# robin-karlsson0/pc-accumulation-lib

Measured on AMD Instinct MI355X. Metric: Mpoints/s projected+accumulated and BEV frames/s @256x256; 1/2/4/8 GPU, higher is better.
Workload: dtype f64; 1 GPU; KITTI-360 single forward cam, 120k pts/frame, 200 m horizon (~201 live frames, 5169634 stored pts), one 256x256x21 BEV per integrated frame; points_per_frame=120000, bev_px=256, view_m=80

## Files before the change

### pc-accumulation-lib_amd/csrc/pca_api.hip

```cpp
#include <stdio.h>
#include <cmath>
#include "pca_common.h"

__global__ __launch_bounds__(256) void pca_fetch_block_kernel(const uint4 *src, uint4 *dst, int64_t n16)
{
    for (int64_t i = (int64_t)blockIdx.x * 256 + threadIdx.x; i < n16; i += (int64_t)gridDim.x * 256) dst[i] = src[i];
}

int pca_fetch_block(pca_ctx *ctx, const void *mapped_host, int64_t offset, void *dev, int64_t bytes, hipStream_t s)
{
    if (bytes <= 0) return 0;
    void *src = nullptr;
    PCA_CHECK(ctx, hipHostGetDevicePointer(&src, const_cast<void *>(mapped_host), 0));
    src = reinterpret_cast<char *>(src) + offset;
    const int64_t n16 = (bytes + 15) / 16;
    const int grid = (int)((n16 + 255) / 256 < 64 ? (n16 + 255) / 256 : 64);
    hipLaunchKernelGGL(pca_fetch_block_kernel, dim3(grid), dim3(256), 0, s, reinterpret_cast<const uint4 *>(src),
                       reinterpret_cast<uint4 *>(dev), n16);
    PCA_CHECK(ctx, hipGetLastError());
    return 0;
}

int pca_ctx_reserve_tiles(pca_ctx *ctx, int64_t tiles, hipStream_t s)
{
// ... 107 lines not shown
                    const double ua = s * (row[0] * cone[0] + row[1] * cone[1] + row[2] * cone[2] + q[axis]);
                    bool out = ua >= h;
                    for (int k = 0; k < 4 && out; ++k) {
                        const double *d = cone + 3 + 3 * k;
                        out = s * (row[0] * d[0] + row[1] * d[1] + row[2] * d[2]) >= 0.0;
                    }
                    if (out) return false;
                }
                if (box) {
                    const float *b = box + 6 * (size_t)f;
                    if (b[0] <= b[1] && b[2] <= b[3] && b[4] <= b[5]) {
                        double lo = s * q[axis];
                        for (int c = 0; c < 3; ++c) {
                            const double x0 = s * row[c] * (double)b[2 * c], x1 = s * row[c] * (double)b[2 * c + 1];
                            lo += x0 < x1 ? x0 : x1;
                        }
                        if (lo >= h) return false;
                    }
                }
            }
        return true;
    };
    int a = 0, b = F - 1;
    while (a <= b && !visible(a)) ++a;
    while (b >= a && !visible(b)) --b;
    if (a > b) { *first = -1; *last = -1; } else { *first = a; *last = b; }
    return 0;
}

int pca_bev_view_hint(pca_ctx *ctx, int slot0, int F, const double *then, const float *box, const double *cone, const double now[12],
                      const pca_bev_params *prm)
{
    if (!ctx) return -1;
    int first = 0, last = 0;
    if (pca_host_view_hull(F, then, box, cone, now, prm, &first, &last)) return -1;
    if (first == 0 && last == F - 1) return 0;
    if (first < 0) { first = 0; last = -1; }
    ctx->bin_first = slot0 + first; ctx->bin_end = slot0 + last + 1; ctx->bin_valid = true;
    return 1;
}

int pca_bev_bin_range(pca_ctx *ctx, int slot_first, int slot_last_plus1)
{
    if (!ctx) return -1;
    ctx->bin_first = slot_first; ctx->bin_end = slot_last_plus1; ctx->bin_valid = slot_last_plus1 >= slot_first;
    return 0;
}

static inline bool box_inside(double x, double y, double lo, double hi) { return lo < x && x < hi && lo < y && y < hi; }

int pca_host_ego_to_grid(const double *full, int F, const double R[9], double dx, double dy, double view, int px,
                         double *rows, int32_t *start)
{
    if (F < 2) { if (F == 1 && start) start[0] = 0; return 0; }
    const double h = 0.5 * view, lo = -h, pxd = (double)px, half_px = 0.5 * pxd;
    auto rot = [&](const double *p, double &x, double &y, double &z) {
        x = fma(R[2], p[2], fma(R[1], p[1], R[0] * p[0])) + dx;
        y = fma(R[5], p[2], fma(R[4], p[1], R[3] * p[0])) + dy;
        z = fma(R[8], p[2], fma(R[7], p[1], R[6] * p[0]));
    };
    auto emit = [&](int m, double x, double y, double z) {
        rows[3 * m + 0] = floor(x / view * pxd + half_px);
        rows[3 * m + 1] = floor(y / view * pxd + half_px);
        rows[3 * m + 2] = z;
    };
    int m = 0;
// ... 151 lines not shown
```

### pc-accumulation-lib_amd/csrc/pca_bev.hip

```cpp
#include "pca_bev_common.h"
#include "pca_k1_body.h"
#include <cstdlib>
#include <mutex>

#define KEY_INVALID 0xffffffffu
#define TS 8
#define TCELLS (TS * TS)
#define NFK (2 * TCELLS)
#ifndef AB_THREADS
#define AB_THREADS 1024
#endif
#define MAX_G 512
#ifndef BIN_RUNR
#define BIN_RUNR 4
#endif
#ifndef BIN_WPE
#define BIN_WPE 4
#endif
#ifndef BIN_UNR
#define BIN_UNR 4
#endif
#ifndef BIN_REG_P
#define BIN_REG_P 12
#endif
// ... 2 lines not shown
#endif
#define C_WAVES (C_THREADS / 64)
#define C_HIST_WAVES 4
#define RGB_CAP 4096
#define CONTIG_MIN 2560
#define HEAVY_MIN_DEFAULT 2560
#define FLAG_ROAD (1u << 24)
#define FLAG_DYNOBJ (1u << 25)

struct __attribute__((aligned(16))) RecF { double z; uint32_t iw; uint32_t cw; };
struct RecD { double z; double inten; uint32_t c; uint32_t fk; };

struct alignas(16) BevArgs {
    pca_store st;
    const double *intensity64;
    const int64_t *frame_off;
    int slot_begin, slot_split, slot_end;
    int64_t max_points;
    pca_bev_params prm;
    int n_pend;
    int write_back;
    int pend_slot_end[PCA_BEV_MAX_CHAIN];
    Mat34 pend_T[PCA_BEV_MAX_CHAIN];
    int tx, T, G;
    int Gr, Gp;
    int tile_mult;
    int heavy_min;
    int stagger;
    uint32_t *key;
    uint32_t *bh;
    uint32_t *boff;
    int Gk;
    int bin_first, bin_end;
    int k1_slot, k1_n;
    uint32_t *bh0;
    int split;
    uint32_t *heavy_hint;
    uint32_t heavy_hint_known;
    uint32_t *span_hint;
    uint32_t span_hint_known;
    int heavy_launched;
    uint32_t *heavy;
    void *recs;
    double *planes;
    uint16_t *planes_f16;
    double *extra;
    uint32_t *status;
    int dbg;
    int band_r0, band_rows;
};
#define HQ_CLASSES 32
#define HQ_CURSOR 32
#define HQ_DONE 33
#define HQ_IDS 64

struct Window { int64_t lo, hi, sp, c_lo, c_hi; };

__device__ __forceinline__ int chunk_index(const BevArgs &a, int64_t lo, int64_t sp, int64_t chunk)
{
    (void)a; (void)lo; (void)sp; (void)chunk;
    return (int)blockIdx.x;
}
#define K1_SEG 4096
#define K1_RIDE 32
__device__ __forceinline__ int64_t window_end(const BevArgs &a)
{
// ... 167 lines not shown
    const int gp = table_pos(a, g);
    uint32_t sum = 0;
    if (split) { for (int k = 0; k < per; ++k) sum += t0 + k < a.T ? s_h[2 * (t0 + k)] + s_h[2 * (t0 + k) + 1] : 0u; }
    else { for (int k = 0; k < per; ++k) sum += t0 + k < a.T ? s_h[t0 + k] : 0u; }
    const int lane = threadIdx.x & 63, wave = threadIdx.x >> 6;
    const uint32_t inc = wave_incl_scan_add(sum);
    if (lane == 63) s_wsum[wave] = inc;
    __syncthreads();
    uint32_t before = 0;
    for (int k = 0; k < wave; ++k) before += s_wsum[k];
    uint32_t run = before + inc - sum;
    for (int k = 0; k < per; ++k) {
        const int t = t0 + k;
        if (t >= a.T) break;
        if (split) {
            const uint32_t c0 = s_h[2 * t], c1 = s_h[2 * t + 1];
            s_cur[2 * t] = run;
            s_cur[2 * t + 1] = run + c0;
            a.bh[(int64_t)t * a.Gr + gp] = c0 + c1;
            a.boff[(int64_t)t * a.Gr + gp] = run;
            a.bh0[(int64_t)t * a.Gr + gp] = c0;
            run += c0 + c1;
        } else {
            const uint32_t c = s_h[t];
            s_cur[t] = run;
            a.bh[(int64_t)t * a.Gr + gp] = c;
            a.boff[(int64_t)t * a.Gr + gp] = run;
            run += c;
        }
    }
}
}

template <bool I64, bool BAND = false>
__device__ __forceinline__ void bev_tile_bin_body(const BevArgs &a)
{
    constexpr int REG_P = I64 ? 0 : BIN_REG_P;
    constexpr int UNR = BIN_RUNR;
    extern __shared__ uint32_t s_lds[];
    __shared__ uint32_t s_wsum[AB_THREADS / 64];
    __shared__ uint32_t s_dyn[8];
    uint32_t *s_h = s_lds;
    if (threadIdx.x < 8) {
        uint32_t w = (uint32_t)a.prm.dynobj_mask[0];
#pragma unroll
        for (int i = 1; i < 8; ++i) w = (int)threadIdx.x == i ? (uint32_t)(a.prm.dynobj_mask[i >> 1] >> (32 * (i & 1))) : w;
        s_dyn[threadIdx.x] = w;
    }
    BIN_STAMP(0);
    int g;
    const Window w = chunk_of(a, g);
    const int64_t chunk = seg_stride(w.hi - w.lo, a.G - a.Gk);
    const bool split = bev_split(a, w.hi - w.lo);
    const int hs = split ? 6 : 7;
    const int n_hist = split ? 2 * a.T : a.T;
    uint32_t *s_cur = s_lds + n_hist;
    if ((int)blockIdx.x == a.Gk) {
        const int64_t end_ub = a.Gk ? a.frame_off[a.k1_slot] + a.k1_n : a.frame_off[a.slot_end];
        if (threadIdx.x == 0 && end_ub - a.frame_off[a.slot_begin] > a.max_points + a.k1_n) pca_raise(a.status, PCA_STATUS_STORE_OVERFLOW);
        if (threadIdx.x < HQ_IDS) a.heavy[threadIdx.x] = 0;
        if (threadIdx.x == 0 && a.span_hint) {
            const uint32_t kp = (uint32_t)((w.hi - w.lo + 1023) >> 10);
            if (kp != a.span_hint_known) *a.span_hint = kp;
        }
    }
    for (int t = threadIdx.x; t < n_hist; t += AB_THREADS) s_h[t] = 0;
// ... 140 lines not shown
    BIN_STAMP(4);
    const bool stale = a.n_pend > 0 && !a.write_back;
    for (int64_t base = reg_hi + threadIdx.x; base < w.c_hi; base += MUNR * AB_THREADS) {
        uint32_t key[MUNR], pos[MUNR], rgbs[MUNR];
        double zz[MUNR], iv[MUNR], xs[MUNR], ys[MUNR];
#pragma unroll
        for (int u = 0; u < MUNR; ++u) {
            const int64_t p = base + u * AB_THREADS;
            key[u] = p < w.c_hi ? a.key[p - w.lo] : KEY_INVALID;
        }
#pragma unroll
        for (int u = 0; u < MUNR; ++u) {
            const int64_t p = base + u * AB_THREADS;
            const bool ok = key[u] != KEY_INVALID;
            rgbs[u] = ok ? a.st.rgbs[p] : 0u;
            zz[u] = ok ? a.st.z[p] : 0.0;
            xs[u] = (ok && stale) ? a.st.x[p] : 0.0;
            ys[u] = (ok && stale) ? a.st.y[p] : 0.0;
            if (I64) iv[u] = ok ? a.intensity64[p] : 0.0;
            else iv[u] = ok ? (double)a.st.intensity[p] : 0.0;
        }
#pragma unroll
        for (int u = 0; u < MUNR; ++u) {
            const int64_t p = base + u * AB_THREADS;
            const bool ok = key[u] != KEY_INVALID;
            if (ok && stale) apply_owed(a, pend_hi, p, xs[u], ys[u], zz[u]);
            pos[u] = ok ? seg + atomicAdd(&s_cur[key[u] >> hs], 1u) : 0u;
        }
#pragma unroll
        for (int u = 0; u < MUNR; ++u)
            if (key[u] != KEY_INVALID) bin_store<I64>(a, s_dyn, pos[u], key[u], rgbs[u], zz[u], iv[u], (float)iv[u]);
    }
    BIN_STAMP(5);
    if ((a.dbg & 32) && threadIdx.x == 0 && blockIdx.x < 1024) { g_dbg_stamps[blockIdx.x][6] = (unsigned long long)a.n_pend * 2 + a.write_back; g_dbg_stamps[blockIdx.x][7] = __smid(); }
}

struct RecMap {
    uint32_t pre[1024 + 1];
    uint32_t base[1024];
    uint32_t wsum[16];
};
__device__ __forceinline__ uint32_t recmap_build(RecMap &M, const BevArgs &a, int tile, int nthreads, uint16_t *owner = nullptr, int half = -1)
{
    const int per = (a.Gr + nthreads - 1) / nthreads;
    const int g0 = threadIdx.x * per;
    const uint32_t *cnt = a.bh + (int64_t)tile * a.Gr, *off = a.boff + (int64_t)tile * a.Gr;
    uint32_t c[4] = {0, 0, 0, 0}, o[4] = {0, 0, 0, 0}, c0[4] = {0, 0, 0, 0}, sum = 0;
    int grp[4] = {0, 0, 0, 0};
#pragma unroll
    for (int k = 0; k < 4; ++k)
        if (k < per && g0 + k < a.Gr) {
            grp[k] = table_group(a, g0 + k);
            if (grp[k] < a.G) {
                c[k] = cnt[g0 + k]; o[k] = off[g0 + k];
                if (half >= 0) c0[k] = a.bh0[(int64_t)tile * a.Gr + g0 + k];
            }
        }
    const int64_t lo = window_begin(a), hi0 = window_end(a);
    const int64_t n = hi0 - lo > a.max_points ? a.max_points : hi0 - lo;
    if (half >= 0 && bev_split(a, n)) {
#pragma unroll
        for (int k = 0; k < 4; ++k) { if (half == 0) c[k] = c0[k]; else { o[k] += c0[k]; c[k] -= c0[k]; } }
    }
    const uint32_t chunk = (uint32_t)seg_stride(n, a.G - a.Gk);
#pragma unroll
    for (int k = 0; k < 4; ++k)
// ... 948 lines not shown
#define BAND_TILES 16384
static inline int band_rows(int px) { const int tx = tiles_x(px); return tx * tx <= BAND_TILES ? tx : BAND_TILES / tx; }
static int bev_tile_mult(int Tp)
{
    auto gcd = [](int x, int y) { while (y) { const int t = x % y; x = y; y = t; } return x; };
    int m = (int)(Tp * 0.6180339887) | 1;
    while (m > 1 && gcd(m, Tp) != 1) m -= 2;
    return m < 1 ? 1 : m;
}
static void bev_set_band(BevArgs &a, int r0)
{
    const int rows = band_rows(a.prm.px);
    a.band_r0 = r0;
    a.band_rows = a.tx - r0 < rows ? a.tx - r0 : rows;
    a.T = a.band_rows * a.tx;
    a.tile_mult = bev_tile_mult(a.T);
}
static inline int max_groups()
{
    const char *e = getenv("PCA_BEV_G");
    const int max_g = e ? atoi(e) : MAX_G;
    return (max_g < 1 || max_g > 1024) ? MAX_G : max_g;
}
static inline int n_groups(int64_t max_points)
{
    const char *c = getenv("PCA_BEV_CHUNK");
    const int max_g = max_groups();
    int per_g = c ? atoi(c) : 8192;
    if (per_g < 1024) per_g = 8192;
    int64_t g = (max_points + per_g - 1) / per_g;
    return (int)(g < 1 ? 1 : (g > max_g ? max_g : g));
}

extern "C" {

int64_t pca_bev_workspace_bytes(int64_t max_points, int px)
{
    if (max_points < 1) max_points = 1;
    const int64_t T = (int64_t)band_rows(px) * tiles_x(px), G = n_groups(max_points);
    return align256(max_points * 4) + 3 * align256((G + K1_RIDE + 8) * T * 4) + align256((HQ_IDS + HQ_CLASSES * T) * 4) +
           align256((max_points + G + K1_RIDE + K1_SEG) * 24) + 512;
}

int pca_bev_generate(pca_ctx *ctx, const pca_store *store, const double *intensity64, const int64_t *frame_off,
                     int slot_begin, int slot_split, int slot_end, int64_t max_points, const pca_bev_params *prm,
                     const double *pending_T, int pending_slot_end, void *workspace, int64_t workspace_bytes,
                     double *planes, uint16_t *planes_f16, void *stream)
{
    return pca_bev_generate_ex(ctx, store, intensity64, frame_off, slot_begin, slot_split, slot_end, max_points, prm,
                               pending_T, pending_slot_end, workspace, workspace_bytes, planes, planes_f16, nullptr, stream);
}

int pca_bev_generate_ex(pca_ctx *ctx, const pca_store *store, const double *intensity64, const int64_t *frame_off,
                        int slot_begin, int slot_split, int slot_end, int64_t max_points, const pca_bev_params *prm,
                        const double *pending_T, int pending_slot_end, void *workspace, int64_t workspace_bytes,
                        double *planes, uint16_t *planes_f16, double *extra_planes, void *stream)
{
    const int n = (pending_T && pending_slot_end > slot_begin) ? 1 : 0;
    return pca_bev_generate_chain(ctx, store, intensity64, frame_off, slot_begin, slot_split, slot_end, max_points, prm,
                                  pending_T, &pending_slot_end, n, 1, workspace, workspace_bytes, planes, planes_f16,
                                  extra_planes, stream);
}

static void bev_table_order(BevArgs &a)
{
    static int xt = -1;
// ... 20 lines not shown
    if (!(slot_begin <= slot_split && slot_split <= slot_end)) { ctx->err = "bev: need slot_begin <= slot_split <= slot_end"; return -1; }
    if (max_points >= (1ll << 32)) { ctx->err = "bev: window too large for 32-bit positions"; return -1; }
    if (workspace_bytes < pca_bev_workspace_bytes(max_points, prm->px)) { ctx->err = "bev: workspace too small"; return -1; }
    a.st = *store;
    a.intensity64 = intensity64;
    a.frame_off = frame_off;
    a.slot_begin = slot_begin; a.slot_split = slot_split; a.slot_end = slot_end;
    a.max_points = max_points;
    a.prm = *prm;
    a.n_pend = n_pending;
    a.write_back = write_back ? 1 : 0;
    for (int k = 0; k < PCA_BEV_MAX_CHAIN; ++k) {
        a.pend_slot_end[k] = slot_begin;
        for (int i = 0; i < 12; ++i) a.pend_T[k].m[i] = 0.0;
        if (k >= n_pending) continue;
        if (pending_slot_ends[k] > slot_end) { ctx->err = "bev: a pending slot end lies beyond the window"; return -1; }
        if (k > 0 && pending_slot_ends[k] < pending_slot_ends[k - 1]) { ctx->err = "bev: pending slot ends must ascend"; return -1; }
        a.pend_slot_end[k] = pending_slot_ends[k];
        for (int i = 0; i < 12; ++i) a.pend_T[k].m[i] = pending_Ts[16 * k + i];
    }
    a.tx = tiles_x(prm->px);
    a.band_rows = band_rows(prm->px);
    a.band_r0 = 0;
    a.T = a.band_rows * a.tx;
    a.G = n_groups(max_points);
    bev_table_order(a);
    char *w = reinterpret_cast<char *>((reinterpret_cast<uintptr_t>(workspace) + 255) & ~(uintptr_t)255);
    a.key = reinterpret_cast<uint32_t *>(w); w += align256(max_points * 4);
    a.bh = reinterpret_cast<uint32_t *>(w); w += align256((int64_t)(a.G + K1_RIDE + 8) * a.T * 4);
    a.boff = reinterpret_cast<uint32_t *>(w); w += align256((int64_t)(a.G + K1_RIDE + 8) * a.T * 4);
    a.bh0 = reinterpret_cast<uint32_t *>(w); w += align256((int64_t)(a.G + K1_RIDE + 8) * a.T * 4);
    a.split = 0;
    a.Gk = 0; a.k1_slot = -1; a.k1_n = 0;
    a.bin_first = slot_begin; a.bin_end = slot_end;
    a.heavy = reinterpret_cast<uint32_t *>(w); w += align256((int64_t)(HQ_IDS + HQ_CLASSES * (int64_t)a.T) * 4);
    a.recs = w;
    a.planes = planes;
    a.planes_f16 = planes_f16;
    a.extra = extra_planes;
    { static int hm = -1; if (hm < 0) { const char *e = getenv("PCA_BEV_HEAVY_MIN"); hm = e ? atoi(e) : HEAVY_MIN_DEFAULT; if (hm < 1 || hm > RGB_CAP) hm = RGB_CAP; } a.heavy_min = hm; }
    { static int dbg = -1; if (dbg < 0) { const char *e = getenv("PCA_BEV_DBG"); dbg = e ? atoi(e) : 0; } a.dbg = dbg; }
    { static int sg = -1; if (sg < 0) { const char *e = getenv("PCA_BEV_STAGGER"); sg = e ? atoi(e) : 0; if (sg < 0 || sg > 64) sg = 0; } a.stagger = sg; }
    a.status = ctx->ticket + 1;
    a.tile_mult = bev_tile_mult((a.tx & 3) == 0 ? a.T / 4 : a.T);
    a.heavy_hint = nullptr; a.heavy_hint_known = 0; a.heavy_launched = 1;
    a.span_hint = nullptr; a.span_hint_known = 0;
    return 0;
}

static int bev_set_lds_attributes(pca_ctx *ctx)
{
    static bool lds_set = false;
    if (lds_set) return 0;
#define PCA_BEV_LDS_ATTR(k, bytes) PCA_CHECK(ctx, hipFuncSetAttribute(reinterpret_cast<const void *>(&(k)), hipFuncAttributeMaxDynamicSharedMemorySize, (int)(bytes)))
#define PCA_BEV_HEAVY_ATTR(I) PCA_BEV_LDS_ATTR((bev_tile_cells_heavy<I, false, false>), HEAVY_LDS_BYTES); PCA_BEV_LDS_ATTR((bev_tile_cells_heavy<I, false, true>), HEAVY_LDS_BYTES); \
    PCA_BEV_LDS_ATTR((bev_tile_cells_heavy<I, true, false>), HEAVY_LDS_BYTES); PCA_BEV_LDS_ATTR((bev_tile_cells_heavy<I, true, true>), HEAVY_LDS_BYTES)
    PCA_BEV_HEAVY_ATTR(false);
    PCA_BEV_HEAVY_ATTR(true);
#undef PCA_BEV_HEAVY_ATTR
    PCA_BEV_LDS_ATTR(bev_tile_cells_heavy_many<false>, HEAVY_LDS_BYTES);
    PCA_BEV_LDS_ATTR(bev_tile_cells_heavy_many<true>, HEAVY_LDS_BYTES);
    PCA_BEV_LDS_ATTR(bev_tile_bin_k1, 80 * 1024);
    PCA_BEV_LDS_ATTR(bev_tile_bin<false>, 128 * 1024);
    PCA_BEV_LDS_ATTR(bev_tile_bin<true>, 128 * 1024);
    PCA_BEV_LDS_ATTR(bev_tile_bin_many<false>, 128 * 1024);
    PCA_BEV_LDS_ATTR(bev_tile_bin_many<true>, 128 * 1024);
    PCA_BEV_LDS_ATTR((bev_tile_cells_heavy_band<false, false>), HEAVY_LDS_BYTES);
// ... 54 lines not shown
                           const double *pending_Ts, const int *pending_slot_ends, int n_pending, int write_back,
                           void *workspace, int64_t workspace_bytes, double *planes, uint16_t *planes_f16,
                           double *extra_planes, void *stream)
{
    if (!ctx) return -1;
    const bool bin_given = ctx->bin_valid;
    const int bin_first = ctx->bin_first, bin_end = ctx->bin_end;
    ctx->bin_valid = false;
    if (max_points < 1) max_points = 1;
    hipStream_t s = (hipStream_t)stream;
    PCA_CHECK(ctx, hipSetDevice(ctx->device));
    BevArgs a;
    if (bev_prepare(ctx, store, intensity64, frame_off, slot_begin, slot_split, slot_end, max_points, prm, pending_Ts,
                    pending_slot_ends, n_pending, write_back, workspace, workspace_bytes, planes, planes_f16, extra_planes, a))
        return -1;
    if (bev_set_lds_attributes(ctx)) return -1;
    if (a.band_rows < a.tx) return bev_generate_banded(ctx, a, bin_given, bin_first, bin_end, s);
    const int heavy_grid = a.T < ctx->n_cu ? a.T : ctx->n_cu;
    a.heavy_hint = ctx->heavy_hint_dev;
    a.heavy_hint_known = *ctx->heavy_hint;
    if (a.heavy_hint_known != 0) ctx->heavy_cooldown = 64;
    else if (ctx->heavy_cooldown > 0) --ctx->heavy_cooldown;
    a.heavy_launched = a.heavy_hint_known != 0 || ctx->heavy_cooldown > 0;
    { static int always = -1; if (always < 0) { const char *e = getenv("PCA_BEV_HEAVY_ALWAYS"); always = e ? atoi(e) : 0; } if (always) a.heavy_launched = 1; }
    { static int sp = -1; if (sp < 0) { const char *e = getenv("PCA_BEV_SPLIT"); sp = e ? atoi(e) : 1; }
      a.split = (sp && a.heavy_launched && !intensity64 && (size_t)a.T * 16 <= 128 * 1024) ? (sp == 2 ? 2 : 1) : 0; }
    const size_t lds = (size_t)a.T * 8 * (a.split ? 2 : 1);
    int one_round = 0;
    if (bin_given) {
        static int cu = -1;
        static int64_t pts = -1;
        if (cu < 0) { const char *e = getenv("PCA_BEV_CULL"); cu = e ? atoi(e) : 1; }
        if (pts < 0) { const char *e = getenv("PCA_BEV_ONE_ROUND_PTS"); pts = e ? atoll(e) : 14500; }
        if (cu && !(n_pending > 0 && write_back)) {
            int f = bin_first > slot_begin ? bin_first : slot_begin, e = bin_end < slot_end ? bin_end : slot_end;
            if (e < f) e = f;
            a.bin_first = f; a.bin_end = e;
            a.span_hint = ctx->heavy_hint_dev + 1;
            a.span_hint_known = ctx->heavy_hint[1];
            if (pts > 0 && a.span_hint_known != 0 && (int64_t)a.span_hint_known * 1024 <= pts * ctx->n_cu && a.G > ctx->n_cu) one_round = ctx->n_cu;
        }
    }
    bool fuse = false;
    K1Args k1a;
    if (ctx->k1_pend.valid) {
        static int fk = -1;
        if (fk < 0) { const char *e = getenv("PCA_FUSE_K1"); fk = e ? atoi(e) : 1; }
        const pca_ctx::K1Pending &pd = ctx->k1_pend;
        int nt = 0;
        bool owed_ok = true;
        for (int k = 0; k < n_pending; ++k) owed_ok = owed_ok && pending_slot_ends[k] <= pd.slot;
        fuse = fk && owed_ok && !intensity64 && pd.stream == s && pd.slot == slot_end - 1 && pd.slot >= slot_begin && pd.frame_off == frame_off &&
               pd.store.x == store->x && lds <= 80 * 1024 && pd.fr.n <= K1_RIDE * K1_SEG && pd.fr.n <= max_points &&
               pca_k1_prepare_pending(ctx, &k1a, &nt, s) == 0 && nt <= K1_RIDE;
        { static int fd = -1; if (fd < 0) { const char *e = getenv("PCA_FUSE_DBG"); fd = e ? atoi(e) : 0; }
          if (fd && !fuse)
              fprintf(stderr, "bev: K1 of slot %d not taken along: switch %d owed_ok %d i64 %d stream %d slot %d (window %d..%d) frame_off %d store %d lds %zu n %d max_points %lld nt %d\n",
                      pd.slot, fk, (int)owed_ok, intensity64 != nullptr, pd.stream == s, pd.slot == slot_end - 1, slot_begin, slot_end,
                      pd.frame_off == frame_off, pd.store.x == store->x, lds, pd.fr.n, (long long)max_points, nt); }
        if (fuse) {
            const int cap = max_groups(), G0 = a.G;
            if (one_round) one_round -= nt;
            a.G = one_round > 0 ? one_round + nt : (G0 + nt <= cap || (cap - 2 * nt) * 4 < 3 * G0) ? G0 + nt : cap - nt;
            a.Gk = nt; bev_table_order(a); a.k1_slot = pd.slot; a.k1_n = pd.fr.n;
            a.max_points = max_points - pd.fr.n;
        }
        else if (pca_k1_flush_pending(ctx)) return -1;
    }
    if (one_round > 0 && !fuse) { a.G = one_round; bev_table_order(a); }
    if (ctx->profiling == 2) pca_prof_begin(ctx, PCA_K_BEV_UNIT, s);
// ... 166 lines not shown
```

### pc-accumulation-lib_amd/csrc/pca_common.h

```cpp
#pragma once
#include <hip/hip_runtime.h>
#include <stddef.h>
#include <stdint.h>
#include <string>
#include <vector>

#include <hip/hip_fp16.h>
#include "../../include/pca.h"
#include "pca_wave.h"

#define PCA_WAVE 64

struct K1Frame {
    const float *pts;
    const uint8_t *rgb, *sem, *sem_gt;
    int32_t n;
    int32_t tile0;
    int32_t qpos0;
    int32_t f;
};

struct pca_ctx {
    int device = 0;
    int n_cu = 256;
// ... 63 lines not shown
    uint32_t *heavy_hint = nullptr;
    uint32_t *heavy_hint_dev = nullptr;
    int bin_first = 0, bin_end = 0;
    bool bin_valid = false;
    struct Ev { hipEvent_t a, b; int kid; };
    int profiling = 0;
    std::vector<Ev> evs;
    std::vector<Ev> free_evs;
    double prof_ms[PCA_K_COUNT] = {0};
    int64_t prof_n[PCA_K_COUNT] = {0};
};

void pca_prof_begin(pca_ctx *ctx, int kid, hipStream_t s);
void pca_prof_end(pca_ctx *ctx, hipStream_t s);
#define PCA_LAUNCH_SHM(ctx, kid, kernel, grid, block, shm, stream, ...)        \
    do {                                                                        \
        if ((ctx)->profiling == 1) pca_prof_begin((ctx), (kid), (stream));      \
        hipLaunchKernelGGL(kernel, grid, block, shm, stream, __VA_ARGS__);      \
        if ((ctx)->profiling == 1) pca_prof_end((ctx), (stream));               \
    } while (0)
#define PCA_LAUNCH(ctx, kid, kernel, grid, block, stream, ...) \
    PCA_LAUNCH_SHM(ctx, kid, kernel, grid, block, 0, stream, __VA_ARGS__)

#define PCA_CHECK(ctx, expr)                                                                   \
    do {                                                                                       \
        hipError_t _e = (expr);                                                                \
        if (_e != hipSuccess) {                                                                \
            (ctx)->err = std::string(#expr) + ": " + hipGetErrorString(_e);                    \
            return -1;                                                                         \
        }                                                                                      \
    } while (0)

int pca_k1_flush_pending(pca_ctx *ctx);
int pca_fetch_block(pca_ctx *ctx, const void *mapped_host, int64_t offset, void *dev, int64_t bytes, hipStream_t s);
int pca_ctx_reserve_tiles(pca_ctx *ctx, int64_t tiles, hipStream_t s);
uint32_t pca_ctx_next_epoch(pca_ctx *ctx, hipStream_t s);

struct Mat34 { double m[12]; };
struct Mat44 { double m[16]; };
struct ClassMask { uint64_t w[4]; };

__device__ __forceinline__ bool in_mask(const ClassMask &m, unsigned c)
{
    const unsigned w = c >> 6;
    uint64_t v = m.w[0];
    v = w == 1 ? m.w[1] : v;
    v = w == 2 ? m.w[2] : v;
    v = w == 3 ? m.w[3] : v;
    return (v >> (c & 63)) & 1ull;
}

__device__ __forceinline__ double row4(const double *r, double x, double y, double z)
{
    double a = r[0] * x;
    a = fma(r[1], y, a);
    a = fma(r[2], z, a);
    a = fma(r[3], 1.0, a);
    return a;
}

struct Bilin { double u0, u1, v0, v1, w_ff, w_cc, w_cf, w_fc; };
template <bool STRICT>
__device__ __forceinline__ Bilin bilin_weights(double u, double v)
{
    Bilin b;
    b.u0 = floor(u); b.v0 = floor(v);
// ... 166 lines not shown
```

### pc-accumulation-lib_amd/csrc/pca_session.hip

```cpp
#include <vector>

#include "pca_common.h"

int pca_stage_copy(const void *const *src, void *const *dst, const int64_t *bytes, int n);

static inline int64_t up256(int64_t v) { return (v + 255) & ~255ll; }

extern "C" {

int pca_kitti_integrate(pca_ctx *ctx, const pca_kitti_obs *obs, const double P[12], int H, int W,
                        const uint64_t filter_mask[4], const pca_store *store, int64_t *frame_off, int slot, int sample_mode,
                        pca_host_track *track, const double *T_new_prev, double horizon, int64_t *evicted,
                        double *path_length, void *stream)
{
    if (!ctx) return -1;
    if (!obs || obs->n < 0 || !P || !filter_mask || !store || !frame_off) { ctx->err = "kitti_integrate: bad arguments"; return -1; }
    if (track && (!T_new_prev || !evicted || !path_length)) { ctx->err = "kitti_integrate: the pose track needs T_new_prev and its outputs"; return -1; }
    hipStream_t s = (hipStream_t)stream;
    PCA_CHECK(ctx, hipSetDevice(ctx->device));
    if (pca_k1_flush_pending(ctx)) return -1;
    const void *in[4] = {obs->pts, obs->rgb, obs->sem, obs->sem_gt};
    const int64_t size[4] = {16ll * obs->n, 3ll * H * W, 1ll * H * W, 1ll * obs->n};
    const void *dev[4] = {in[0], in[1], in[2], in[3]};
    int64_t off[4] = {0, 0, 0, 0}, total = 0;
// ... 43 lines not shown
                       obs->n <= (1 << 20);
    if (ctx->k1_defer && plain) {
        pca_ctx::K1Pending &pd = ctx->k1_pend;
        pd.fr = fr;
        for (int i = 0; i < 12; ++i) pd.P[i] = P[i];
        pd.H = H; pd.W = W;
        for (int i = 0; i < 4; ++i) pd.filt[i] = filter_mask[i];
        pd.store = *store; pd.frame_off = frame_off; pd.slot = slot; pd.sample_mode = sample_mode; pd.stream = s;
        pd.stage_idx = slot_st ? (int)(slot_st - ctx->stage) : -1;
        pd.valid = true;
    } else {
        const int rc = pca_kitti_project_sample_filter_ex(ctx, &fr, 1, P, H, W, filter_mask, store, frame_off, slot, sample_mode, stream);
        if (slot_st) {
            const hipError_t e = hipEventRecord(slot_st->done, s);
            if (e == hipSuccess) slot_st->busy = true;
            else {
                (void)hipStreamSynchronize(s);
                if (rc == 0) { ctx->err = std::string("kitti_integrate: hipEventRecord(stage done): ") + hipGetErrorString(e); return -1; }
            }
        }
        if (rc != 0) return rc;
    }
    if (track) *evicted = pca_host_track_step(track, T_new_prev, horizon, path_length);
    return 0;
}

int pca_kitti_generate_bev(pca_ctx *ctx, const pca_store *store, const int64_t *frame_off, int slot_begin, int slot_split,
                           int slot_end, int64_t max_points, const pca_bev_params *prm, const double *pending_Ts,
                           const int *pending_slot_ends, int n_pending, int write_back, void *workspace,
                           int64_t workspace_bytes, uint16_t *planes_f16, void *host_planes, const pca_host_track *track,
                           double *traj_rows, int32_t *traj_start, int32_t *n_rows, void *stream)
{
    if (!ctx) return -1;
    if (!prm || !planes_f16 || !track || !traj_rows || !traj_start || !n_rows) { ctx->err = "kitti_generate_bev: bad arguments"; return -1; }
    const int64_t F = pca_host_track_len(track);
    if (F != slot_end - slot_begin) { ctx->err = "kitti_generate_bev: the pose track and the window disagree about the number of frames"; return -1; }
    static thread_local std::vector<double> rel;
    rel.resize((size_t)(3 * (F > 0 ? F : 1)));
    const double *Hp = pca_host_track_poses(track);
    for (int64_t f = 0; f < F; ++f)
        for (int k = 0; k < 3; ++k) rel[(size_t)(3 * f + k)] = Hp[4 * f + k] - prm->origin[k];
    *n_rows = pca_host_ego_to_grid(rel.data(), (int)F, prm->R, prm->dx, prm->dy, prm->view, prm->px, traj_rows, traj_start);
    if (pca_bev_generate_chain(ctx, store, nullptr, frame_off, slot_begin, slot_split, slot_end, max_points, prm, pending_Ts,
                               pending_slot_ends, n_pending, write_back, workspace, workspace_bytes, nullptr, planes_f16,
                               nullptr, stream) != 0)
        return -1;
    if (!host_planes) return 0;
    return pca_host_d2h_async(ctx, planes_f16, host_planes, 21ll * prm->px * prm->px * 2, stream);
}

int pca_kitti_integrate_v(pca_ctx *ctx, pca_kitti_integrate_args *a)
{
    if (!ctx) return -1;
    if (!a) { ctx->err = "kitti_integrate_v: no argument block"; return -1; }
    return pca_kitti_integrate(ctx, a->obs, a->P, a->H, a->W, a->filter_mask, a->store, a->frame_off, a->slot, a->sample_mode,
                               a->track, a->T_new_prev, a->horizon, &a->evicted, &a->path_length, a->stream);
}

int pca_kitti_generate_bev_v(pca_ctx *ctx, pca_kitti_generate_bev_args *a)
{
    if (!ctx) return -1;
    if (!a) { ctx->err = "kitti_generate_bev_v: no argument block"; return -1; }
    a->hinted = 0;
    if (a->hint_F > 0 && !(a->n_pending > 0 && a->write_back)) {
        const int rc = pca_bev_view_hint(ctx, a->hint_slot0, a->hint_F, a->hint_then, a->hint_box, a->hint_cone, a->hint_now, a->prm);
        if (rc < 0) { ctx->err = "kitti_generate_bev_v: bad view hint"; return -1; }
        a->hinted = rc;
    }
    return pca_kitti_generate_bev(ctx, a->store, a->frame_off, a->slot_begin, a->slot_split, a->slot_end, a->max_points, a->prm,
                                  a->pending_Ts, a->pending_slot_ends, a->n_pending, a->write_back, a->workspace,
                                  a->workspace_bytes, a->planes_f16, a->host_planes, a->track, a->traj_rows, a->traj_start,
                                  &a->n_rows, a->stream);
}

}
```

### pc-accumulation-lib_amd/pca_amd/device_store.py

```python
import ctypes as C
import os

import numpy as np
import torch

from . import _lib
from ._lib import PcaBevParams, PcaKittiFrame, PcaStore

CULL = os.environ.get('PCA_BEV_CULL', '1') != '0'


class DeviceStore:
    CHAIN_MAX = 4
    CHAIN_K = int(os.environ.get('PCA_BEV_CHAIN', '4'))

    def __init__(self, capacity=1 << 24, max_frames=4096, device=None, intensity_div255=False):
        self.ctx = _lib.Context.get(device)
        self.device = torch.device('cuda', self.ctx.device_index)
        self.intensity_div255 = bool(intensity_div255)
        self.max_frames = int(max_frames)
        self._alloc(int(capacity))
        self.frame_off = torch.zeros(self.max_frames + 1, dtype=torch.int64, device=self.device)
        self._moved = np.eye(4)
        self.cull = CULL
        self.hints_taken = 0
        self._alloc_frame_tables(self.max_frames)
        self.head = 0
        self.tail = 0
        self.ub_tail = 0
        self.lb_head = 0
        self._ub = []
        self._ub_sum = 0
        self._pending = []
        self._k1_cache = None
        self._k1_src = None
        self._ia = None
        self._ws = None
        self._ws_many = None
        self._ws_points, self._ws_px = 0, 0
        self._dedup_ws = None
        self._obs_out = None
        self._k1_noted = None
# ... 65 lines not shown
                if self._box_pin is None or self._box_pin.shape[0] < self.frame_box.shape[0]:
                    self._box_pin = torch.empty(tuple(self.frame_box.shape), dtype=torch.int32, pin_memory=True)
                self._box_pin[:n].copy_(self.frame_box[self.head:self.tail], non_blocking=True)
                ev = torch.cuda.Event()
                ev.record()
                self._box_copy = (ev, self.head, n)
                self._since_box = 0

    def _poll_boxes(self):
        if self._box_copy is None or not self._box_copy[0].query():
            return
        _, first, n = self._box_copy
        self._box_copy = None
        rows = self._box_pin[:n].numpy()
        dec = np.empty((n, 6), dtype=np.float32)
        self.ctx.lib.pca_f32_box_decode(rows.ctypes.data, n, dec.ctypes.data)
        known = dec[:, 0] <= dec[:, 1]
        tgt = self._box[first:first + n]
        tgt[known] = dec[known]

    def view_hint_into(self, args, first_frame, last_frame):
        n = last_frame - first_frame
        if not self.cull or n < 4:
            return 0
        a = self.head + first_frame
        args.hint_slot0 = a
        args.hint_then, args.hint_box = self._then_addr + 96 * a, self._box_addr + 24 * a
        args.hint_cone = self._cone[2] if (self._cone is not None and self._n_nocone == 0) else None
        args.hint_now = self._moved.ctypes.data
        return n

    def view_hint(self, prm, first_frame, last_frame, write_back):
        n = last_frame - first_frame
        if not self.cull or write_back or n < 4:
            return 0
        a = self.head + first_frame
        cone = self._cone[2] if (self._cone is not None and self._n_nocone == 0) else None
        return self._count_hint(self.ctx.lib.pca_bev_view_hint(self.ctx.h, a, n, self._then_addr + 96 * a, self._box_addr + 24 * a, cone,
                                              self._moved.ctypes.data, C.addressof(prm)))

    def _count_hint(self, r):
        self.hints_taken += 1 if r > 0 else 0
        return r

    def c_store(self):
        if self._cstore is None:
            self._cstore = PcaStore(self.x.data_ptr(), self.y.data_ptr(), self.z.data_ptr(), self.intensity.data_ptr(),
                                    self.rgbs.data_ptr(), self.inst.data_ptr(), self.dyn.data_ptr(), self.capacity,
                                    self.frame_box.data_ptr())
        return self._cstore

    @property
    def n_frames(self):
        return self.tail - self.head

    def set_defer_k1(self, on):
        self.ctx.check(self.ctx.lib.pca_k1_defer(self.ctx.h, 1 if on else 0))
        self.ctx.k1_defer = bool(on)
        if not on:
            self._k1_noted = None

    def flush_k1(self):
        if self._k1_noted is not None:
            self.ctx.check(self.ctx.lib.pca_k1_flush(self.ctx.h))
            self._k1_noted = None

    def __del__(self):
# ... 442 lines not shown
```

Baseline: 1439 Mpoints/s.

## Enable view culling during pending write-back by streaming culled frames' pose updates

View-hull culling used to be turned off whenever pending pose transforms had to be written back, so every stored point went through binning. Now culling stays on in that case. Bin blocks handle only the visible frame range, then split the remaining out-of-view points among themselves and apply the owed transforms in a lightweight streaming loop that writes x/y/z back. This adds a per-block tail pass over the culled points, guarded by an env switch, and resets bin_valid on error paths.

```diff
diff --git a/pc-accumulation-lib_amd/csrc/pca_api.hip b/pc-accumulation-lib_amd/csrc/pca_api.hip
--- a/pc-accumulation-lib_amd/csrc/pca_api.hip
+++ b/pc-accumulation-lib_amd/csrc/pca_api.hip
@@ -163,6 +163,7 @@
                       const pca_bev_params *prm)
 {
     if (!ctx) return -1;
+    ctx->bin_valid = false;
     int first = 0, last = 0;
     if (pca_host_view_hull(F, then, box, cone, now, prm, &first, &last)) return -1;
     if (first == 0 && last == F - 1) return 0;
diff --git a/pc-accumulation-lib_amd/csrc/pca_bev.hip b/pc-accumulation-lib_amd/csrc/pca_bev.hip
--- a/pc-accumulation-lib_amd/csrc/pca_bev.hip
+++ b/pc-accumulation-lib_amd/csrc/pca_bev.hip
@@ -58,6 +58,7 @@
     uint32_t *boff;
     int Gk;
     int bin_first, bin_end;
+    int wb_rest;
     int k1_slot, k1_n;
     uint32_t *bh0;
     int split;
@@ -291,6 +292,42 @@
 }
 }
 
+__device__ __forceinline__ void bin_stream_rest(const BevArgs &a, int g)
+{
+    constexpr int U = 2;
+    const int e = a.Gk ? a.k1_slot : a.slot_end;
+    const int64_t p0 = a.frame_off[a.slot_begin];
+    if (a.frame_off[e] - p0 > a.max_points) return;
+    const int64_t n0 = a.frame_off[a.bin_first] - p0;
+    const int64_t p1 = a.frame_off[a.bin_end < e ? a.bin_end : e];
+    const int64_t n1 = p1 < a.frame_off[e] ? a.frame_off[e] - p1 : 0;
+    const int P = a.G - a.Gk;
+    const int64_t n = n0 + n1, share = (n + P - 1) / P;
+    const int64_t lo = (int64_t)(g - a.Gk) * share, hi = lo + share < n ? lo + share : n;
+    PendHi ph;
+#pragma unroll
+    for (int k = 0; k < PCA_BEV_MAX_CHAIN; ++k)
+        ph.v[k] = (k < a.n_pend && a.pend_slot_end[k] > a.slot_begin) ? a.frame_off[a.pend_slot_end[k]] : p0;
+    for (int64_t base = lo + threadIdx.x; base < hi; base += U * AB_THREADS) {
+        double X[U], Y[U], Z[U];
+        int64_t pp[U];
+#pragma unroll
+        for (int u = 0; u < U; ++u) {
+            const int64_t i = base + u * AB_THREADS;
+            const int64_t p = i >= hi ? p0 : (i < n0 ? p0 + i : p1 + (i - n0));
+            pp[u] = i < hi ? p : -1;
+            X[u] = a.st.x[p];
+            Y[u] = a.st.y[p];
+            Z[u] = a.st.z[p];
+        }
+#pragma unroll
+        for (int u = 0; u < U; ++u)
+            if (pp[u] >= 0 && apply_owed(a, ph, pp[u], X[u], Y[u], Z[u])) {
+                a.st.x[pp[u]] = X[u]; a.st.y[pp[u]] = Y[u]; a.st.z[pp[u]] = Z[u];
+            }
+    }
+}
+
 template <bool I64, bool BAND = false>
 __device__ __forceinline__ void bev_tile_bin_body(const BevArgs &a)
 {
@@ -497,6 +534,7 @@
             if (key[u] != KEY_INVALID) bin_store<I64>(a, s_dyn, pos[u], key[u], rgbs[u], zz[u], iv[u], (float)iv[u]);
     }
     BIN_STAMP(5);
+    if (!BAND && a.wb_rest) bin_stream_rest(a, g);
     if ((a.dbg & 32) && threadIdx.x == 0 && blockIdx.x < 1024) { g_dbg_stamps[blockIdx.x][6] = (unsigned long long)a.n_pend * 2 + a.write_back; g_dbg_stamps[blockIdx.x][7] = __smid(); }
 }
 
@@ -1511,6 +1549,13 @@
     return (int)(g < 1 ? 1 : (g > max_g ? max_g : g));
 }
 
+int pca_bev_wb_visible()
+{
+    static int v = -1;
+    if (v < 0) { const char *e = getenv("PCA_BEV_WB_VISIBLE"); v = e ? (atoi(e) != 0) : 1; }
+    return v;
+}
+
 extern "C" {
 
 int64_t pca_bev_workspace_bytes(int64_t max_points, int px)
@@ -1597,7 +1642,7 @@
     a.bh0 = reinterpret_cast<uint32_t *>(w); w += align256((int64_t)(a.G + K1_RIDE + 8) * a.T * 4);
     a.split = 0;
     a.Gk = 0; a.k1_slot = -1; a.k1_n = 0;
-    a.bin_first = slot_begin; a.bin_end = slot_end;
+    a.bin_first = slot_begin; a.bin_end = slot_end; a.wb_rest = 0;
     a.heavy = reinterpret_cast<uint32_t *>(w); w += align256((int64_t)(HQ_IDS + HQ_CLASSES * (int64_t)a.T) * 4);
     a.recs = w;
     a.planes = planes;
@@ -1718,10 +1763,11 @@
         static int64_t pts = -1;
         if (cu < 0) { const char *e = getenv("PCA_BEV_CULL"); cu = e ? atoi(e) : 1; }
         if (pts < 0) { const char *e = getenv("PCA_BEV_ONE_ROUND_PTS"); pts = e ? atoll(e) : 14500; }
-        if (cu && !(n_pending > 0 && write_back)) {
+        if (cu && (!(n_pending > 0 && write_back) || pca_bev_wb_visible())) {
             int f = bin_first > slot_begin ? bin_first : slot_begin, e = bin_end < slot_end ? bin_end : slot_end;
             if (e < f) e = f;
             a.bin_first = f; a.bin_end = e;
+            a.wb_rest = n_pending > 0 && write_back;
             a.span_hint = ctx->heavy_hint_dev + 1;
             a.span_hint_known = ctx->heavy_hint[1];
             if (pts > 0 && a.span_hint_known != 0 && (int64_t)a.span_hint_known * 1024 <= pts * ctx->n_cu && a.G > ctx->n_cu) one_round = ctx->n_cu;
diff --git a/pc-accumulation-lib_amd/csrc/pca_common.h b/pc-accumulation-lib_amd/csrc/pca_common.h
--- a/pc-accumulation-lib_amd/csrc/pca_common.h
+++ b/pc-accumulation-lib_amd/csrc/pca_common.h
@@ -119,6 +119,7 @@
     } while (0)
 
 int pca_k1_flush_pending(pca_ctx *ctx);
+int pca_bev_wb_visible();
 int pca_fetch_block(pca_ctx *ctx, const void *mapped_host, int64_t offset, void *dev, int64_t bytes, hipStream_t s);
 int pca_ctx_reserve_tiles(pca_ctx *ctx, int64_t tiles, hipStream_t s);
 uint32_t pca_ctx_next_epoch(pca_ctx *ctx, hipStream_t s);
diff --git a/pc-accumulation-lib_amd/csrc/pca_session.hip b/pc-accumulation-lib_amd/csrc/pca_session.hip
--- a/pc-accumulation-lib_amd/csrc/pca_session.hip
+++ b/pc-accumulation-lib_amd/csrc/pca_session.hip
@@ -99,9 +99,9 @@
                            double *traj_rows, int32_t *traj_start, int32_t *n_rows, void *stream)
 {
     if (!ctx) return -1;
-    if (!prm || !planes_f16 || !track || !traj_rows || !traj_start || !n_rows) { ctx->err = "kitti_generate_bev: bad arguments"; return -1; }
+    if (!prm || !planes_f16 || !track || !traj_rows || !traj_start || !n_rows) { ctx->bin_valid = false; ctx->err = "kitti_generate_bev: bad arguments"; return -1; }
     const int64_t F = pca_host_track_len(track);
-    if (F != slot_end - slot_begin) { ctx->err = "kitti_generate_bev: the pose track and the window disagree about the number of frames"; return -1; }
+    if (F != slot_end - slot_begin) { ctx->bin_valid = false; ctx->err = "kitti_generate_bev: the pose track and the window disagree about the number of frames"; return -1; }
     static thread_local std::vector<double> rel;
     rel.resize((size_t)(3 * (F > 0 ? F : 1)));
     const double *Hp = pca_host_track_poses(track);
@@ -129,9 +129,10 @@
     if (!ctx) return -1;
     if (!a) { ctx->err = "kitti_generate_bev_v: no argument block"; return -1; }
     a->hinted = 0;
-    if (a->hint_F > 0 && !(a->n_pending > 0 && a->write_back)) {
+    ctx->bin_valid = false;
+    if (a->hint_F > 0 && (!(a->n_pending > 0 && a->write_back) || pca_bev_wb_visible())) {
         const int rc = pca_bev_view_hint(ctx, a->hint_slot0, a->hint_F, a->hint_then, a->hint_box, a->hint_cone, a->hint_now, a->prm);
-        if (rc < 0) { ctx->err = "kitti_generate_bev_v: bad view hint"; return -1; }
+        if (rc < 0) { ctx->bin_valid = false; ctx->err = "kitti_generate_bev_v: bad view hint"; return -1; }
         a->hinted = rc;
     }
     return pca_kitti_generate_bev(ctx, a->store, a->frame_off, a->slot_begin, a->slot_split, a->slot_end, a->max_points, a->prm,
diff --git a/pc-accumulation-lib_amd/pca_amd/device_store.py b/pc-accumulation-lib_amd/pca_amd/device_store.py
--- a/pc-accumulation-lib_amd/pca_amd/device_store.py
+++ b/pc-accumulation-lib_amd/pca_amd/device_store.py
@@ -8,6 +8,7 @@
 from ._lib import PcaBevParams, PcaKittiFrame, PcaStore
 
 CULL = os.environ.get('PCA_BEV_CULL', '1') != '0'
+WB_VISIBLE = os.environ.get('PCA_BEV_WB_VISIBLE', '1') != '0'
 
 
 class DeviceStore:
@@ -139,7 +140,7 @@
 
     def view_hint(self, prm, first_frame, last_frame, write_back):
         n = last_frame - first_frame
-        if not self.cull or write_back or n < 4:
+        if not self.cull or (write_back and not WB_VISIBLE) or n < 4:
             return 0
         a = self.head + first_frame
         cone = self._cone[2] if (self._cone is not None and self._n_nocone == 0) else None
```

Result: no change. 1437 Mpoints/s, median of 2 (-0.2%).
